# Jannertje/spacetime-fullgrid-parallel

Hardware: AMD Instinct MI355X
Metric: Kronecker-matvec GB/s (algorithmic bytes; share of 8 TB/s HBM peak in roofline.frac) + PCG iters/s, J_time=6 J_space=9 square (higher is better)
Workload: dtype f64; 1 GPU; y = (A_t kron M_x + M_t kron A_x) x, P1 on the uniform interval x P1 on the red-refined square, x ~ U[0,1) seed 128; J_space=9, N=65, M=1046529, nnz_M_x=7317521, nnz_A_x=5228553, parallelism=time-slab x1

## Files before the change

include/stk.h:

```cpp
#ifndef STK_H
#define STK_H

#include <stdint.h>

#ifdef __cplusplus
extern "C" {
#endif

const char *stk_last_error(void);
int stk_version(void);
int stk_device_info(int32_t *n_cu, int32_t *wave_size, int64_t *hbm_bytes);
int stk_set_tuning(const char *key, int32_t value);

int stk_slab_gather_columns(void *stream, int32_t M, int32_t n_cols,
                            const int32_t *cols, const double *x, int32_t ld_x,
                            double *y, int32_t ld_y);
int stk_slab_scatter_columns(void *stream, int32_t M, int32_t n_cols,
                             const int32_t *cols, const double *x, int32_t ld_x,
                             double *y, int32_t ld_y);

int stk_slab_ld(int32_t n_loc);
int stk_slab_alloc(int32_t M, int32_t n_loc, int32_t *ld, double **slab);
int stk_slab_free(double *slab);
int stk_slab_upload(void *stream, int32_t M, int32_t n_loc, int32_t ld,
// ... 298 lines not shown
    const int32_t *fwd_rows;
    int32_t n_bwd;
    const int32_t *bwd_ptr_host;
    const int32_t *bwd_rows;
    const int32_t *p_indptr, *p_indices;
    const double *p_vals;
    const int32_t *r_indptr, *r_indices;
    const double *r_vals;
    const stk_ell_rows *ell_a, *ell_fwd, *ell_bwd, *ell_p, *ell_r;
    const int32_t *fwd_pos_host, *bwd_pos_host;
    const stk_ell_rows *ell_ra;
    const stk_ell_rows *ell_fwd0;
    int32_t n_tile_rows;
    const int32_t *fwd_tile_row_host, *bwd_tile_row_host;
    const stk_ell_rows *ell_fwd_alt, *ell_bwd_alt;
} stk_mg_level;

typedef struct stk_mg stk_mg;

int stk_mg_create(int32_t n_levels, const stk_mg_level *levels_host,
                  int32_t smoothsteps, int32_t vcycles, int32_t n_kinds,
                  const double *coarse_inv, int32_t max_ld, stk_mg **out);
int stk_mg_destroy(stk_mg *mg);
int stk_mg_set_option(stk_mg *plan, const char *key, int32_t value);
int stk_mg_apply(stk_mg *mg, void *stream, int32_t n_loc, int32_t ld,
                 double ca, const double *cm, const int32_t *kind,
                 const double *f, double *u);
int stk_mg_coarse_levels(const stk_mg *plan);
int stk_mg_set_member_matrices(stk_mg *plan, int32_t level, int32_t n_kinds,
                               const int32_t *const *indptr_host,
// ... 119 lines not shown
```

spacetime-fullgrid-parallel_amd/csrc/mg.hip:

```cpp
#include <algorithm>
#include <cstdio>
#include <cstdlib>
#include <cstring>
#include <map>
#include <vector>

#include "stk_common.h"

namespace {

constexpr int GBS = 256;

__global__ __launch_bounds__(GBS) void gs_group_kernel(int64_t total, const int32_t *__restrict__ rows,
                                                       int32_t n_loc, int32_t ld,
                                                       const int32_t *__restrict__ indptr,
                                                       const int32_t *__restrict__ indices,
                                                       const double *__restrict__ va, double ca,
                                                       const double *__restrict__ vm,
                                                       const double *__restrict__ cm,
                                                       const int32_t *__restrict__ diag,
                                                       const double *__restrict__ f, double *u, int diag_free)
{
    const int64_t stride = (int64_t)gridDim.x * GBS;
    for (int64_t idx = (int64_t)blockIdx.x * GBS + threadIdx.x; idx < total; idx += stride) {
// ... 39 lines not shown

}

constexpr int64_t COARSE_MAX_ROWS = 4096;

struct EllLevel {
    bool has_a = false, has_gs = false, has_p = false, has_r = false, has_ra = false, has_alt = false;
    bool ra_rows_as_r = false;
    stk_ell_rows a, fwd, bwd, p, r, ra;
    stk_ell_rows fwd_alt, bwd_alt;
    std::vector<stk_ell_rows> fwd0;
    std::vector<int32_t> fwd_pos, bwd_pos;
    std::vector<int32_t> fwd_trow, bwd_trow;
    int n_tile_rows = 0;
    mutable std::map<int, std::vector<int32_t>> fwd_strips, bwd_strips;
};

struct stk_mg {
    std::vector<stk_mg_level> lv;
    std::vector<EllLevel> ell;
    std::vector<std::vector<int32_t>> fwd_ptr, bwd_ptr;
    int smoothsteps, vcycles, n_kinds, max_ld;
    const double *coarse_inv;
    std::vector<double *> u, f, r;
    stk_coarse_plan *coarse = nullptr;
    int Lc = -1;
    std::vector<void *> adopted;
    int fuse_restrict = -1;
    int fuse_min_level = 0, fuse_max_level = 1 << 30;
    int fast_until_cycle = 0;
    int fast_parts = 0;
    int strip_pct = 100;
};

static inline bool ell_slab_ok(int64_t rows, int ld)
{
    return (ld & 1) == 0 && rows * ld * 8 < ((int64_t)1 << 36);
}

static bool can_zero_start(const stk_mg *mg, int level, int ld)
{
    const EllLevel &E = mg->ell[level];
    return stk_tune(g_tuning.mg_zero_start) && level >= 1 && mg->smoothsteps >= 1 && E.has_gs && !E.fwd0.empty() &&
           E.fwd0.size() + 1 == E.fwd_pos.size() && ell_slab_ok(mg->lv[level].n, ld);
}

static const std::vector<int32_t> *strip_table(const EllLevel &E, bool backward, int64_t rows, int ld, int its,
// ... 8 lines not shown
    const int T = E.n_tile_rows, span = T + Q - 1;
    const int strip_width = stk_tune(g_tuning.mg_strip_width);
    const int min_width = strip_width > 0 ? strip_width * Q : 2;
    if (S > span / min_width) S = span / min_width;
    if (S < 2) return nullptr;
    auto &cache = backward ? E.bwd_strips : E.fwd_strips;
    const int key = S * 1024 + its;
    auto it = cache.find(key);
    if (it != cache.end()) return &it->second;
    const std::vector<int32_t> &tr = backward ? E.bwd_trow : E.fwd_trow;
    std::vector<int32_t> tab((size_t)S * Q * 2);
    for (int s = 0; s < S; ++s)
        for (int q = 0; q < Q; ++q) {
            const int g = q % ng;
            const int32_t *b = tr.data() + pos[g], *e = tr.data() + pos[g + 1];
            const int lo_row = (int)((int64_t)s * span / S) - q, hi_row = (int)((int64_t)(s + 1) * span / S) - q;
            const int32_t *lo = (s == 0) ? b : std::lower_bound(b, e, lo_row);
            const int32_t *hi = (s == S - 1) ? e : std::lower_bound(b, e, hi_row);
            tab[((size_t)s * Q + q) * 2] = (int32_t)(lo - tr.data());
            tab[((size_t)s * Q + q) * 2 + 1] = (int32_t)(hi - tr.data());
        }
    return &cache.emplace(key, std::move(tab)).first->second;
}

static int smooth_level(stk_mg *mg, hipStream_t st, int level, int n_loc, int ld, double ca, const double *cm,
                        int its, bool backward, const double *f, double *u, bool zero_start = false, int cycle = 1 << 30)
{
    const stk_mg_level &L = mg->lv[level];
    const EllLevel &E = mg->ell[level];
    if (E.has_gs && ell_slab_ok(L.n, ld)) {
        const bool alt = E.has_alt && cycle < mg->fast_until_cycle;
        const stk_ell_rows &e = alt ? (backward ? E.bwd_alt : E.fwd_alt) : (backward ? E.bwd : E.fwd);
        const std::vector<int32_t> &pos = backward ? E.bwd_pos : E.fwd_pos;
        const int ng = (int)pos.size() - 1;
        const bool zs = zero_start && !backward && its >= 1;
        const std::vector<int32_t> *strips =
            strip_table(E, backward, L.n, ld, its, stk_tune(g_tuning.mg_strip_mb) * (mg->strip_pct / 100.0));
        const int S = strips ? (int)(strips->size() / (2 * (size_t)ng * its)) : 1;
        const int Q = its * ng;
        for (int s = 0; s < S; ++s)
            for (int q = 0; q < Q; ++q) {
                const int g = q % ng;
                const int p0 = strips ? (*strips)[((size_t)s * Q + q) * 2] : pos[g];
                const int p1 = strips ? (*strips)[((size_t)s * Q + q) * 2 + 1] : pos[g + 1];
                if (strips) g_tuning.mg_strips_used.fetch_add(1, std::memory_order_relaxed);
                int rc;
                if (zs && q < ng) {
                    rc = stk_rows_ell_launch(st, 1, &E.fwd0[g], p0 - pos[g], p1 - pos[g], n_loc, ld, L.n, L.n, ca, cm,
                                             g == 0 ? f : u, 0.0, 0.0, f, u, 1);
                } else {
                    rc = stk_rows_ell_launch(st, 1, &e, p0, p1, n_loc, ld, L.n, L.n, ca, cm, u, 0.0, 0.0, f, u);
                }
                if (rc) return rc;
            }
        return 0;
    }
    const std::vector<int32_t> &ptr = backward ? mg->bwd_ptr[level] : mg->fwd_ptr[level];
    const int32_t *rows = backward ? L.bwd_rows : L.fwd_rows;
    const int ngroups = (int)ptr.size() - 1;
    for (int it = 0; it < its; ++it) {
        for (int g = 0; g < ngroups; ++g) {
            const int nr = ptr[g + 1] - ptr[g];
            if (nr == 0) continue;
            const int64_t total = (int64_t)nr * n_loc;
            hipLaunchKernelGGL(gs_group_kernel, dim3(stk_flat_grid(total, GBS)), dim3(GBS), 0, st, total,
                               rows + ptr[g], n_loc, ld, L.indptr, L.indices, L.vals_a, ca,
                               cm ? L.vals_m : nullptr, cm, L.diag, f, u, E.has_gs ? E.fwd.diag_free : 1);
            STK_LAUNCH_CHECK();
        }
    }
    return 0;
// ... 12 lines not shown
    if (u_zero && j >= 1 && !zero_start) {
        const int cols = std::min(ld, (n_loc + 1) & ~1);
        if (cols == ld)
            STK_HIP(hipMemsetAsync(u_j, 0, sizeof(double) * (size_t)L.n * ld, st));
        else
            STK_HIP(hipMemset2DAsync(u_j, sizeof(double) * (size_t)ld, 0, sizeof(double) * (size_t)cols, (size_t)L.n,
                                     st));
    }
    if (j == 0) {
        const int total = L.n * n_loc;
        hipLaunchKernelGGL(coarse_kernel, dim3((total + GBS - 1) / GBS), dim3(GBS), 0, st, L.n, n_loc, ld,
                           mg->coarse_inv, cm ? 1.0 : 1.0 / ca, cm ? kind : nullptr, f_j, u_j);
        STK_LAUNCH_CHECK();
        return 0;
    }
    int rc = smooth_level(mg, st, j, n_loc, ld, ca, cm, mg->smoothsteps, false, f_j, u_j, zero_start,
                          (mg->fast_parts & 1) ? -1 : cycle);
    if (rc) return rc;
    const stk_mg_level &C = mg->lv[j - 1];
    double *r_j = mg->r[j], *d_c = mg->f[j - 1], *u_c = mg->u[j - 1];
    const EllLevel &E = mg->ell[j];
    const bool even = ell_slab_ok(L.n, ld);
    const bool fuse_restrict = (mg->fuse_restrict >= 0 ? mg->fuse_restrict != 0 : stk_tune(g_tuning.mg_fuse_restrict) != 0) &&
                               ((j >= mg->fuse_min_level && j <= mg->fuse_max_level) || cycle < mg->fast_until_cycle ||
                                (mg->fast_parts & 2));
    if (fuse_restrict && E.has_ra && E.has_r && even) {
        const int one_pass = stk_tune(g_tuning.mg_restrict_one_pass);
        rc = (one_pass && E.ra_rows_as_r && (cm != nullptr || one_pass >= 2))
                 ? stk_rows_ell2_launch(st, &E.ra, &E.r, n_loc, ld, L.n, C.n, ca, cm, u_j, f_j, d_c)
                 : -1;
        if (rc == -1) {
            rc = stk_rows_ell_launch(st, 0, &E.r, 0, E.r.n_pos, n_loc, ld, L.n, C.n, 1.0, nullptr, f_j, 1.0, 0.0,
                                     nullptr, d_c);
            if (rc) return rc;
            rc = stk_rows_ell_launch(st, 0, &E.ra, 0, E.ra.n_pos, n_loc, ld, L.n, C.n, ca, cm, u_j, 1.0, -1.0, d_c,
                                     d_c);
        }
        if (rc) return rc;
    } else {
        if (E.has_a && even)
            rc = stk_rows_ell_launch(st, 0, &E.a, 0, E.a.n_pos, n_loc, ld, L.n, L.n, ca, cm, u_j, 1.0, -1.0, f_j,
                                     r_j);
        else
            rc = stk_csr_spmm(st, L.n, n_loc, ld, L.indptr, L.indices, L.vals_a, ca, cm ? L.vals_m : nullptr, cm,
                              u_j, 1.0, -1.0, f_j, r_j);
        if (rc) return rc;
        if (E.has_r && even)
            rc = stk_rows_ell_launch(st, 0, &E.r, 0, E.r.n_pos, n_loc, ld, L.n, C.n, 1.0, nullptr, r_j, 1.0, 0.0,
                                     nullptr, d_c);
        else
            rc = stk_csr_spmm(st, C.n, n_loc, ld, L.r_indptr, L.r_indices, L.r_vals, 1.0, nullptr, nullptr, r_j,
                              1.0, 0.0, nullptr, d_c);
        if (rc) return rc;
    }
    rc = mgm(mg, st, j - 1, n_loc, ld, ca, cm, kind, d_c, u_c, true, cycle);
    if (rc) return rc;
    if (E.has_p && even)
        rc = stk_rows_ell_launch(st, 0, &E.p, 0, E.p.n_pos, n_loc, ld, C.n, L.n, 1.0, nullptr, u_c, -1.0, 1.0, u_j,
                                 u_j);
    else
        rc = stk_csr_spmm(st, L.n, n_loc, ld, L.p_indptr, L.p_indices, L.p_vals, 1.0, nullptr, nullptr, u_c, -1.0,
                          1.0, u_j, u_j);
    if (rc) return rc;
    return smooth_level(mg, st, j, n_loc, ld, ca, cm, mg->smoothsteps, true, f_j, u_j, false, cycle);
}

extern "C" int stk_mg_create(int32_t n_levels, const stk_mg_level *levels, int32_t smoothsteps, int32_t vcycles,
                             int32_t n_kinds, const double *coarse_inv, int32_t max_ld, stk_mg **out)
{
    STK_REQUIRE(n_levels >= 1 && levels && out, "stk_mg_create: bad arguments");
    STK_REQUIRE(smoothsteps >= 0 && vcycles >= 1 && max_ld >= 1, "stk_mg_create: bad parameters");
    STK_REQUIRE(coarse_inv && n_kinds >= 1, "stk_mg_create: coarse inverse missing");
    stk_mg *mg = new stk_mg();
    mg->smoothsteps = smoothsteps;
    mg->vcycles = vcycles;
    mg->n_kinds = n_kinds;
    mg->max_ld = max_ld;
    mg->coarse_inv = coarse_inv;
    mg->lv.assign(levels, levels + n_levels);
// ... 26 lines not shown
            E.fwd_pos.assign(L.fwd_pos_host, L.fwd_pos_host + L.n_fwd + 1);
            E.bwd_pos.assign(L.bwd_pos_host, L.bwd_pos_host + L.n_bwd + 1);
            E.has_gs = true;
        }
        if (E.has_gs && L.ell_fwd_alt && L.ell_bwd_alt && L.ell_fwd_alt->n_pos == E.fwd.n_pos &&
            L.ell_bwd_alt->n_pos == E.bwd.n_pos) {
            E.fwd_alt = *L.ell_fwd_alt;
            E.bwd_alt = *L.ell_bwd_alt;
            E.has_alt = true;
        }
        if (E.has_gs && L.n_tile_rows > 1 && L.fwd_tile_row_host && L.bwd_tile_row_host) {
            E.fwd_trow.assign(L.fwd_tile_row_host, L.fwd_tile_row_host + E.fwd.n_pos);
            E.bwd_trow.assign(L.bwd_tile_row_host, L.bwd_tile_row_host + E.bwd.n_pos);
            E.n_tile_rows = L.n_tile_rows;
        }
        mg->lv[j].ell_a = mg->lv[j].ell_fwd = mg->lv[j].ell_bwd = mg->lv[j].ell_p = mg->lv[j].ell_r = nullptr;
        mg->lv[j].ell_ra = mg->lv[j].ell_fwd0 = nullptr;
        mg->lv[j].ell_fwd_alt = mg->lv[j].ell_bwd_alt = nullptr;
    }
    mg->u.assign(n_levels, nullptr);
    mg->f.assign(n_levels, nullptr);
    mg->r.assign(n_levels, nullptr);
    for (int j = 0; j < n_levels; ++j) {
        const stk_mg_level &L = mg->lv[j];
        if (L.n <= 0 || !L.indptr || !L.indices || !L.vals_a || !L.diag) {
            stk_set_error("stk_mg_create: level %d incomplete", j);
            stk_mg_destroy(mg);
            return 2;
        }
        if (j > 0) {
// ... 105 lines not shown
        mg->fuse_min_level = value;
        return 0;
    }
    if (std::strcmp(key, "fuse_restrict_max_level") == 0) {
        mg->fuse_max_level = value;
        return 0;
    }
    if (std::strcmp(key, "fast_until_cycle") == 0) {
        mg->fast_until_cycle = value;
        return 0;
    }
    if (std::strcmp(key, "fast_parts") == 0) {
        mg->fast_parts = value;
        return 0;
    }
    if (std::strcmp(key, "strip_pct") == 0) {
        STK_REQUIRE(value >= 1 && value <= 10000, "stk_mg_set_option: strip_pct=%d not in 1..10000", value);
        mg->strip_pct = value;
        return 0;
    }
    stk_set_error("stk_mg_set_option: unknown key '%s' (fuse_restrict, fuse_restrict_min_level, fuse_restrict_max_level, fast_until_cycle, fast_parts, strip_pct)", key);
    return 2;
}

extern "C" int stk_mg_apply(stk_mg *mg, void *stream, int32_t n_loc, int32_t ld, double ca, const double *cm,
                            const int32_t *kind, const double *f, double *u)
{
    const stk_timed timed_(STK_OP_MULTIGRID, stream);
    STK_REQUIRE(mg && f && u && f != u, "stk_mg_apply: bad pointers");
    STK_REQUIRE(n_loc > 0 && ld >= n_loc && ld <= mg->max_ld, "stk_mg_apply: ld=%d exceeds plan max_ld=%d", ld,
                mg->max_ld);
    STK_REQUIRE(cm == nullptr || mg->lv[0].vals_m != nullptr, "stk_mg_apply: cm given but plan has no vals_m");
    STK_REQUIRE(ca != 0.0 || cm, "stk_mg_apply: zero matrix");
    hipStream_t st = stk_stream(stream);
    const int J = (int)mg->lv.size() - 1;
    for (int v = 0; v < mg->vcycles; ++v) {
// ... 16 lines not shown
```

spacetime-fullgrid-parallel_amd/csrc/rows_ell.hip:

```cpp
#include <cstring>

#include "stk_common.h"

namespace {

constexpr int BS = 512;
enum { MODE_SPMM = 0, MODE_GS = 1 };

struct RowsArgs {
    const int32_t *idx;
    const double *va, *vm;
    const int32_t *row_ids;
    const double *dia_a, *dia_m;
    const double *cm;
    const double *x;
    const double *z;
    double *y;
    double ca, alpha, beta;
    int32_t pos_begin, pos_end;
    int32_t n_loc, ld, P, R;
    int32_t ngroups, chunk;
    int32_t reverse;
    int32_t zero_own;
    uint32_t x_bytes, y_bytes;
// ... 369 lines not shown
        case 9: return launch_npf<MODE, 9, HAS_M>(st, a, grid, lds);
        case 12: return launch_npf<MODE, 12, HAS_M>(st, a, grid, lds);
        case 16: return launch_npf<MODE, 16, HAS_M>(st, a, grid, lds);
        case 20: return launch_npf<MODE, 20, HAS_M>(st, a, grid, lds);
    }
    stk_set_error("rows_ell: K=%d is not one of 2, 4, 5, 6, 7, 9, 12, 16, 20", K);
    return 2;
}

}

int stk_rows_ell_launch(hipStream_t st, int mode, const stk_ell_rows *e, int32_t pos_begin, int32_t pos_end,
                        int32_t n_loc, int32_t ld, int64_t x_rows, int64_t y_rows, double ca, const double *cm,
                        const double *x, double alpha, double beta, const double *z, double *y, int zero_own)
{
    if (pos_end <= pos_begin) return 0;
    STK_REQUIRE(e && e->idx && e->va, "rows_ell: incomplete matrix");
    STK_REQUIRE((cm == nullptr) || e->vm, "rows_ell: cm given but the matrix has no vm");
    STK_REQUIRE(n_loc > 0 && ld >= n_loc && (ld & 1) == 0, "rows_ell: bad n_loc=%d ld=%d (ld must be even)", n_loc,
                ld);
    STK_REQUIRE(x_rows * ld * 8 < ((int64_t)1 << 36) && y_rows * ld * 8 < ((int64_t)1 << 36),
                "rows_ell: slab exceeds 64 GiB");
    STK_REQUIRE((((uintptr_t)x | (uintptr_t)y | (uintptr_t)z) & 15) == 0, "rows_ell: slabs must be 16-byte aligned");
    STK_REQUIRE((n_loc + 1) / 2 <= BS, "rows_ell: n_loc too large");
    RowsArgs a;
    a.idx = e->idx;
    a.va = e->va;
    a.vm = cm ? e->vm : nullptr;
    a.row_ids = e->row_ids;
    a.dia_a = e->dia_a;
    a.dia_m = e->dia_m;
    a.cm = cm;
// ... 5 lines not shown
    a.beta = z ? beta : 0.0;
    a.pos_begin = pos_begin;
    a.pos_end = pos_end;
    a.n_loc = n_loc;
    a.ld = ld;
    a.P = (n_loc + 1) / 2;
    a.R = BS / a.P;
    if (a.R * e->K > 4 * BS) a.R = 4 * BS / e->K;
    a.ngroups = (pos_end - pos_begin + a.R - 1) / a.R;
    a.chunk = (a.ngroups + 7) / 8;
    a.reverse = (int)(g_rows_launch_count++ & 1u);
    a.zero_own = (zero_own || e->diag_free) ? 1 : 0;
    a.wide = stk_tune(g_tuning.rows_force_wide) || x_rows * ld * 8 >= ((int64_t)1 << 32) || y_rows * ld * 8 >= ((int64_t)1 << 32);
    a.x_bytes = a.wide ? 0u : (uint32_t)(x_rows * ld * 8);
    a.y_bytes = a.wide ? 0u : (uint32_t)(y_rows * ld * 8);
    a.nt_store = mode == MODE_GS ? 0 : 1;
    if (mode == MODE_GS) STK_REQUIRE(e->dia_a && (!cm || e->dia_m), "rows_ell: GS needs the diagonal arrays");
    const int K = e->K;
    const int KS = (K + 3) & ~3;
    const bool has_m = cm != nullptr;
    const size_t buf_doubles =
        ((size_t)(has_m ? 2 : 1) * a.R * KS + 2 * a.R + ((size_t)a.R * KS + a.R + 1) / 2 + 2) & ~(size_t)1;
    const size_t lds = 2 * buf_doubles * sizeof(double) + 16;
    const int n_cu = stk_cu_count();
    int per_cu = K >= 12 ? 2 : 3;
    int per_xcd = (n_cu / 8) * per_cu;
    if (per_xcd > a.chunk) per_xcd = a.chunk;
    if (per_xcd < 1) per_xcd = 1;
    const unsigned grid = (unsigned)per_xcd * 8;
    if (mode == MODE_GS)
        return has_m ? launch_k<MODE_GS, true>(st, a, K, grid, lds) : launch_k<MODE_GS, false>(st, a, K, grid, lds);
    return has_m ? launch_k<MODE_SPMM, true>(st, a, K, grid, lds) : launch_k<MODE_SPMM, false>(st, a, K, grid, lds);
}

int stk_rows_ell2_launch(hipStream_t st, const stk_ell_rows *e, const stk_ell_rows *e2, int32_t n_loc, int32_t ld,
                         int64_t x_rows, int64_t y_rows, double ca, const double *cm, const double *x,
                         const double *x2, double *y)
{
    if (e->K != 20 || e2->K != 7 || e->n_pos != e2->n_pos || e->n_pos <= 0) return -1;
    STK_REQUIRE(e->idx && e->va && e2->idx && e2->va, "rows_ell2: incomplete matrix");
    STK_REQUIRE((cm == nullptr) || e->vm, "rows_ell2: cm given but the matrix has no vm");
    STK_REQUIRE(n_loc > 0 && ld >= n_loc && (ld & 1) == 0, "rows_ell2: bad n_loc=%d ld=%d", n_loc, ld);
    STK_REQUIRE(x_rows * ld * 8 < ((int64_t)1 << 36) && y_rows * ld * 8 < ((int64_t)1 << 36), "rows_ell2: slab exceeds 64 GiB");
    STK_REQUIRE((((uintptr_t)x | (uintptr_t)x2 | (uintptr_t)y) & 15) == 0, "rows_ell2: slabs must be 16-byte aligned");
    STK_REQUIRE((n_loc + 1) / 2 <= BS, "rows_ell2: n_loc too large");
    constexpr int K = 20, K2 = 7, KS = 20, KS2 = 8;
    Rows2Args b;
    RowsArgs &a = b.a;
    a.idx = e->idx;
    a.va = e->va;
    a.vm = cm ? e->vm : nullptr;
    a.row_ids = e->row_ids;
    a.dia_a = a.dia_m = nullptr;
    a.cm = cm;
    a.x = x;
    a.z = y;
    a.y = y;
    a.ca = ca;
    a.alpha = 1.0;
    a.beta = 0.0;
    a.pos_begin = 0;
    a.pos_end = e->n_pos;
    a.n_loc = n_loc;
    a.ld = ld;
    a.P = (n_loc + 1) / 2;
    a.R = BS / a.P;
    if (a.R * K > 4 * BS) a.R = 4 * BS / K;
    a.ngroups = (e->n_pos + a.R - 1) / a.R;
    a.chunk = (a.ngroups + 7) / 8;
    a.reverse = (int)(g_rows_launch_count++ & 1u);
    a.zero_own = 0;
    a.wide = stk_tune(g_tuning.rows_force_wide) || x_rows * ld * 8 >= ((int64_t)1 << 32) || y_rows * ld * 8 >= ((int64_t)1 << 32);
    a.x_bytes = a.wide ? 0u : (uint32_t)(x_rows * ld * 8);
    a.y_bytes = a.wide ? 0u : (uint32_t)(y_rows * ld * 8);
    a.nt_store = 0;
    b.idx2 = e2->idx;
    b.va2 = e2->va;
    b.x2 = x2;
    b.x2_bytes = a.x_bytes;
    const bool has_m = cm != nullptr;
    auto lds_of = [&](int R) {
        const size_t val_doubles = (size_t)(has_m ? 2 : 1) * R * KS + (size_t)R * KS2;
        const size_t buf_doubles = (val_doubles + ((size_t)R * KS + (size_t)R * KS2 + R + 1) / 2 + 2) & ~(size_t)1;
        return 2 * buf_doubles * sizeof(double) + 16;
    };
    while (a.R > 1 && lds_of(a.R) > 60 * 1024) --a.R;
    a.ngroups = (e->n_pos + a.R - 1) / a.R;
    a.chunk = (a.ngroups + 7) / 8;
    const size_t lds = lds_of(a.R);
    const int n_cu = stk_cu_count();
    int per_xcd = (n_cu / 8) * 2;
    if (per_xcd > a.chunk) per_xcd = a.chunk;
    if (per_xcd < 1) per_xcd = 1;
    const unsigned grid = (unsigned)per_xcd * 8;
    if (has_m)
        return a.wide ? launch2_npf<K, K2, true, true>(st, b, grid, lds) : launch2_npf<K, K2, true, false>(st, b, grid, lds);
    return a.wide ? launch2_npf<K, K2, false, true>(st, b, grid, lds) : launch2_npf<K, K2, false, false>(st, b, grid, lds);
}

extern "C" int stk_ell_spmm(void *stream, const stk_ell_rows *ell, int32_t n_loc, int32_t ld, int32_t x_rows,
                            double ca, const double *cm, const double *x, double alpha, double beta,
                            const double *z, double *y)
// ... 8 lines not shown
```

spacetime-fullgrid-parallel_amd/source/_lib.py:

```python
import ctypes
import os

import numpy as np
import torch

_HERE = os.path.dirname(os.path.abspath(__file__))
LIB_PATH = os.path.join(os.path.dirname(_HERE), 'libstk.so')

c_i32, c_i64, c_f64, c_p = (ctypes.c_int32, ctypes.c_int64, ctypes.c_double,
                            ctypes.c_void_p)


OPERATOR_FN = ctypes.CFUNCTYPE(ctypes.c_int, ctypes.c_void_p, ctypes.c_void_p,
                               ctypes.c_void_p, ctypes.c_void_p)
ALLREDUCE_FN = ctypes.CFUNCTYPE(ctypes.c_int, ctypes.c_void_p,
                                ctypes.POINTER(ctypes.c_double), ctypes.c_int32)


class EllPattern(ctypes.Structure):
    _fields_ = [('M', c_i32), ('K', c_i32), ('ell_idx', c_p),
                ('row_ids', c_p), ('ovf_indptr', c_p), ('ovf_indices', c_p)]


class KronEllTerm(ctypes.Structure):
# ... 33 lines not shown
                ('n_fwd', c_i32), ('fwd_ptr_host', c_p), ('fwd_rows', c_p),
                ('n_bwd', c_i32), ('bwd_ptr_host', c_p), ('bwd_rows', c_p),
                ('p_indptr', c_p), ('p_indices', c_p), ('p_vals', c_p),
                ('r_indptr', c_p), ('r_indices', c_p), ('r_vals', c_p),
                ('ell_a', ctypes.POINTER(EllRows)),
                ('ell_fwd', ctypes.POINTER(EllRows)),
                ('ell_bwd', ctypes.POINTER(EllRows)),
                ('ell_p', ctypes.POINTER(EllRows)),
                ('ell_r', ctypes.POINTER(EllRows)),
                ('fwd_pos_host', c_p), ('bwd_pos_host', c_p),
                ('ell_ra', ctypes.POINTER(EllRows)),
                ('ell_fwd0', ctypes.POINTER(EllRows)),
                ('n_tile_rows', c_i32), ('fwd_tile_row_host', c_p),
                ('bwd_tile_row_host', c_p),
                ('ell_fwd_alt', ctypes.POINTER(EllRows)),
                ('ell_bwd_alt', ctypes.POINTER(EllRows))]


_PROTOTYPES = {
    'stk_last_error': (ctypes.c_char_p, []),
    'stk_version': (ctypes.c_int, []),
    'stk_device_info': (ctypes.c_int, [c_p, c_p, c_p]),
    'stk_axpby': (ctypes.c_int, [c_p, c_i64, c_f64, c_p, c_f64, c_p]),
    'stk_axpbyz': (ctypes.c_int, [c_p, c_i64, c_f64, c_p, c_f64, c_p, c_p]),
    'stk_dot_work_size': (c_i64, []),
    'stk_dot': (ctypes.c_int, [c_p, c_i64, c_p, c_p, c_p, c_p]),
    'stk_set_tuning': (ctypes.c_int, [ctypes.c_char_p, c_i32]),
    'stk_partition': (ctypes.c_int, [c_i32, c_i32, c_i32, c_p, c_p, c_p, c_p]),
    'stk_pcg_work_size': (c_i64, [c_i64]),
    'stk_pcg_solve': (ctypes.c_int, [
        c_p, c_i64, OPERATOR_FN, c_p, OPERATOR_FN, c_p, ALLREDUCE_FN, c_p, c_p,
# ... 303 lines not shown
```

spacetime-fullgrid-parallel_amd/source/multigrid.py:

```python
import ctypes
import threading

import numpy as np
import scipy.sparse as sp
import torch

from . import _lib
from .assembly import prolongation_matrices
from .linop import (EllRowsMatrix, SpaceOp, tile_order_from_coords,
                    tile_rows_from_coords,
                    union_pattern)


class MeshHierarchy:
    def __init__(self, fes=None, shared_comm=None, P_mats=None):
        self.coords = None
        if P_mats is None:
            mesh = getattr(fes, 'mesh', fes)
            P_mats = prolongation_matrices(mesh)
            self.coords = mesh.points[~mesh.boundary]
        self.shared_comm = shared_comm
        self.P_mats = [sp.csr_matrix(P) for P in P_mats]
        self.R_mats = [P.T.tocsr() for P in self.P_mats]
        self.J = len(self.P_mats)
# ... 17 lines not shown
    def tile_order(self, n):
        if self.coords is None:
            return np.arange(n, dtype=np.int32)
        return self.shared(('tile', n), lambda: tile_order_from_coords(self.coords[:n]))

    def coord_band(self, n):
        if self.coords is None:
            return None

        def make():
            _, band = np.unique(np.round(np.asarray(self.coords)[:n, -1], 12), return_inverse=True)
            return band.astype(np.int64)

        return self.shared(('band', n), make)

    def transfer_copies(self, j):
        def make():
            P = sp.csr_matrix(self.P_mats[j - 1])
            R = sp.csr_matrix(self.R_mats[j - 1])
            dev, ells = {}, {}
            for name, m, order in (('p', P, self.tile_order(P.shape[0])),
                                   ('r', R, self.tile_order(P.shape[1]))):
                m.sort_indices()
                dev[name + '_indptr'] = _lib.to_dev(np.asarray(m.indptr, dtype=np.int32))
                dev[name + '_indices'] = _lib.to_dev(np.asarray(m.indices, dtype=np.int32))
                dev[name + '_vals'] = _lib.to_dev(np.asarray(m.data, dtype=np.float64))
                ells[name] = EllRowsMatrix(m.indptr, m.indices, m.data, None, order)
            return dev, ells

        return self.shared(('transfer', j), make)

    def prepare(self):
        sizes = [P.shape[1] for P in self.P_mats] + ([self.P_mats[-1].shape[0]] if self.P_mats else [])
        for n in reversed(sizes):
            self.tile_order(n)
            self.coord_band(n)
        if _lib.compute_device().type == 'cuda':
            for j in reversed(range(1, self.J + 1)):
                self.transfer_copies(j)
        return self


def _tile_order(hierarchy, n):
    if hasattr(hierarchy, 'tile_order'):
        return hierarchy.tile_order(n)
    coords = getattr(hierarchy, 'coords', None)
    return np.arange(n, dtype=np.int32) if coords is None else tile_order_from_coords(coords[:n])


def _shared(hierarchy, key, make):
    return hierarchy.shared(key, make) if hasattr(hierarchy, 'shared') else make()


def _mat_key(mat):
    return (mat.indptr.ctypes.data, mat.indices.ctypes.data, mat.data.ctypes.data, mat.nnz)


def _drop_roundoff(mat, rel=1e-14):
    if mat.nnz:
        mat.data[np.abs(mat.data) < rel * np.abs(mat.data).max()] = 0.0
        mat.eliminate_zeros()
    return mat
# ... 296 lines not shown
        if self.has_m:
            dev['vals_m'] = _lib.to_dev(vals[1])
        L.n = n
        host = {}
        if j > 0:
            tile = _tile_order(hierarchy, n)
            rank = np.empty(n, dtype=np.int64)
            rank[tile] = np.arange(n)
            band = coupling_bands(hierarchy.coords, indptr, indices, rows_of,
                                  hierarchy.coord_band(n) if hasattr(hierarchy, 'coord_band') else None)
            if band is not None and self.band_merge > 1 and hierarchy.coords is not None:
                band = band // self.band_merge
            key = rank if band is None else band * np.int64(n) + rank
            vm = vals[1] if self.has_m else None
            moved = {}
            transfers = threading.Thread(
                target=_lib.in_device_context(self._transfer_ells),
                args=(j, hierarchy, mats, tile, moved))
            transfers.start()
            ells = {'a': EllRowsMatrix(indptr, indices, vals[0], vm, tile)}
            for name, bw in (('fwd', False), ('bwd', True)):
                ptr, rows = gauss_seidel_schedule(indptr, indices, bw,
                                                  on_device=(dev['indptr'], dev['indices']))
                host[name + '_ptr'] = ptr
                dev[name + '_rows'] = _lib.to_dev(rows)
                setattr(L, 'n_' + name, len(ptr) - 1)
                setattr(L, name + '_ptr_host',
                        ptr.ctypes.data_as(ctypes.c_void_p))
                groups = [rows[ptr[g]:ptr[g + 1]] for g in range(len(ptr) - 1)]
                groups = [r_[np.argsort(key[r_], kind='stable')] for r_ in groups]
                listed = (np.concatenate(groups) if n else
                          np.zeros(0, dtype=np.int64))
                full_rows, alt_copies = self._row_form(j)
                if not full_rows:
                    ells[name] = EllRowsMatrix(indptr, indices, vals[0], vm,
# ... 13 lines not shown
                host[name + '_pos'] = ptr
                setattr(L, name + '_pos_host',
                        ptr.ctypes.data_as(ctypes.c_void_p))
                if not bw:
                    fwd_groups = groups
            transfers.join()
            if 'error' in moved:
                raise moved['error']
            dev.update(moved['dev'])
            ells.update(moved['ells'])
            if all(e.ok for e in ells.values()):
                if moved['ra'].ok:
                    ells['ra'] = moved['ra']
                for name, e in ells.items():
                    setattr(L, 'ell_' + name, ctypes.pointer(e.struct))
                host['ells'] = ells
                self._zero_start_ells(L, host, indptr, indices, vals[0], vm,
                                      diag, fwd_groups)
                EllRowsMatrix.check_all(list(ells.values()) + list(host.get('fwd0', ([],))[0]))
        for name, t in dev.items():
            setattr(L, name, _lib.ptr(t))
        self._keep.append((dev, host))
        if j == self.J:
            self.groups_fwd = len(host['fwd_ptr']) - 1 if j > 0 else 0

    def _transfer_ells(self, j, hierarchy, mats, tile, out):
        try:
            P = sp.csr_matrix(hierarchy.P_mats[j - 1])
            R = sp.csr_matrix(hierarchy.R_mats[j - 1])
            nc = P.shape[1]
            tile_c = _tile_order(hierarchy, nc)

            def transfer_copies():
                dev_, ells_ = {}, {}
                for name, m, order in (('p', P, tile), ('r', R, tile_c)):
                    m.sort_indices()
                    dev_[name + '_indptr'] = _lib.to_dev(np.asarray(m.indptr, dtype=np.int32))
                    dev_[name + '_indices'] = _lib.to_dev(np.asarray(m.indices, dtype=np.int32))
                    dev_[name + '_vals'] = _lib.to_dev(np.asarray(m.data, dtype=np.float64))
                    ells_[name] = EllRowsMatrix(m.indptr, m.indices, m.data, None, order)
                return dev_, ells_

            if hasattr(hierarchy, 'transfer_copies'):
                shared_dev, shared_ells = hierarchy.transfer_copies(j)
            else:
                shared_dev, shared_ells = transfer_copies()
            dev, ells = dict(shared_dev), dict(shared_ells)
            prods = [_shared(hierarchy, ('ra', j, _mat_key(m)),
                             lambda m=m: _drop_roundoff(galerkin_product(R, m, None))) for m in mats]
            ra_ptr, ra_idx, ra_vals = union_pattern(prods)
            out['ra'] = EllRowsMatrix(ra_ptr, ra_idx, ra_vals[0],
                                      ra_vals[1] if self.has_m else None, tile_c)
            out['dev'], out['ells'] = dev, ells
        except Exception as exc:
            out['error'] = exc

    def _zero_start_ells(self, L, host, indptr, indices, va, vm, diag,
                         groups):
        n = len(indptr) - 1
        if not groups or any(len(g) == 0 for g in groups):
            return
        grp = np.empty(n, dtype=np.int64)
        for g, rows in enumerate(groups):
            grp[rows] = g
        rows_of = np.repeat(np.arange(n), np.diff(indptr))
        kept = np.bincount(rows_of[grp[indices] < grp[rows_of]], minlength=n)
        ells = [EllRowsMatrix(indptr, indices, va, vm, rows, pad_col=-1,
# ... 268 lines not shown
```

Baseline: 4264 GB/s.

## Interleave restriction and prolongation with Gauss-Seidel strips for cache reuse

```diff
diff --git a/include/stk.h b/include/stk.h
--- a/include/stk.h
+++ b/include/stk.h
@@ -336,6 +336,7 @@
     int32_t n_tile_rows;
     const int32_t *fwd_tile_row_host, *bwd_tile_row_host;
     const stk_ell_rows *ell_fwd_alt, *ell_bwd_alt;
+    const int32_t *a_ready_host, *r_ready_host, *ra_ready_host, *p_band_host;
 } stk_mg_level;
 
 typedef struct stk_mg stk_mg;
diff --git a/spacetime-fullgrid-parallel_amd/csrc/mg.hip b/spacetime-fullgrid-parallel_amd/csrc/mg.hip
--- a/spacetime-fullgrid-parallel_amd/csrc/mg.hip
+++ b/spacetime-fullgrid-parallel_amd/csrc/mg.hip
@@ -2,10 +2,12 @@
 #include <cstdio>
 #include <cstdlib>
 #include <cstring>
+#include <functional>
 #include <map>
 #include <vector>
 
-#include "stk_common.h"
+#include "mg_strips.h"
+#include "rows_ell.h"
 
 namespace {
 
@@ -77,6 +79,7 @@
     std::vector<int32_t> fwd_trow, bwd_trow;
     int n_tile_rows = 0;
     mutable std::map<int, std::vector<int32_t>> fwd_strips, bwd_strips;
+    std::vector<int32_t> a_ready, r_ready, ra_ready, p_band;
 };
 
 struct stk_mg {
@@ -94,6 +97,7 @@
     int fast_until_cycle = 0;
     int fast_parts = 0;
     int strip_pct = 100;
+    int strip_transfers = 1;
 };
 
 static inline bool ell_slab_ok(int64_t rows, int ld)
@@ -132,7 +136,7 @@
         for (int q = 0; q < Q; ++q) {
             const int g = q % ng;
             const int32_t *b = tr.data() + pos[g], *e = tr.data() + pos[g + 1];
-            const int lo_row = (int)((int64_t)s * span / S) - q, hi_row = (int)((int64_t)(s + 1) * span / S) - q;
+            const int lo_row = stk_strip_edge(s, T, Q, S) - q, hi_row = stk_strip_edge(s + 1, T, Q, S) - q;
             const int32_t *lo = (s == 0) ? b : std::lower_bound(b, e, lo_row);
             const int32_t *hi = (s == S - 1) ? e : std::lower_bound(b, e, hi_row);
             tab[((size_t)s * Q + q) * 2] = (int32_t)(lo - tr.data());
@@ -141,8 +145,22 @@
     return &cache.emplace(key, std::move(tab)).first->second;
 }
 
+static const std::vector<int32_t> *level_strips(const stk_mg *mg, int level, int ld, int its, bool backward)
+{
+    const EllLevel &E = mg->ell[level];
+    if (!E.has_gs || !ell_slab_ok(mg->lv[level].n, ld)) return nullptr;
+    return strip_table(E, backward, mg->lv[level].n, ld, its,
+                       stk_tune(g_tuning.mg_strip_mb) * (mg->strip_pct / 100.0));
+}
+
+struct StripHooks {
+    const std::vector<int32_t> *strips;
+    std::function<int(int, int)> before, after;
+};
+
 static int smooth_level(stk_mg *mg, hipStream_t st, int level, int n_loc, int ld, double ca, const double *cm,
-                        int its, bool backward, const double *f, double *u, bool zero_start = false, int cycle = 1 << 30)
+                        int its, bool backward, const double *f, double *u, bool zero_start = false, int cycle = 1 << 30,
+                        const StripHooks *hooks = nullptr)
 {
     const stk_mg_level &L = mg->lv[level];
     const EllLevel &E = mg->ell[level];
@@ -152,11 +170,14 @@
         const std::vector<int32_t> &pos = backward ? E.bwd_pos : E.fwd_pos;
         const int ng = (int)pos.size() - 1;
         const bool zs = zero_start && !backward && its >= 1;
-        const std::vector<int32_t> *strips =
-            strip_table(E, backward, L.n, ld, its, stk_tune(g_tuning.mg_strip_mb) * (mg->strip_pct / 100.0));
+        const std::vector<int32_t> *strips = hooks ? hooks->strips : level_strips(mg, level, ld, its, backward);
         const int S = strips ? (int)(strips->size() / (2 * (size_t)ng * its)) : 1;
         const int Q = its * ng;
-        for (int s = 0; s < S; ++s)
+        for (int s = 0; s < S; ++s) {
+            if (hooks && hooks->before) {
+                const int rc = hooks->before(s, S);
+                if (rc) return rc;
+            }
             for (int q = 0; q < Q; ++q) {
                 const int g = q % ng;
                 const int p0 = strips ? (*strips)[((size_t)s * Q + q) * 2] : pos[g];
@@ -171,8 +192,14 @@
                 }
                 if (rc) return rc;
             }
-        return 0;
-    }
+            if (hooks && hooks->after) {
+                const int rc = hooks->after(s, S);
+                if (rc) return rc;
+            }
+        }
+        return 0;
+    }
+    STK_REQUIRE(!hooks, "smooth_level: strip hooks on a level without ELL sweeps");
     const std::vector<int32_t> &ptr = backward ? mg->bwd_ptr[level] : mg->fwd_ptr[level];
     const int32_t *rows = backward ? L.bwd_rows : L.fwd_rows;
     const int ngroups = (int)ptr.size() - 1;
@@ -215,47 +242,99 @@
         STK_LAUNCH_CHECK();
         return 0;
     }
-    int rc = smooth_level(mg, st, j, n_loc, ld, ca, cm, mg->smoothsteps, false, f_j, u_j, zero_start,
-                          (mg->fast_parts & 1) ? -1 : cycle);
-    if (rc) return rc;
     const stk_mg_level &C = mg->lv[j - 1];
     double *r_j = mg->r[j], *d_c = mg->f[j - 1], *u_c = mg->u[j - 1];
     const EllLevel &E = mg->ell[j];
     const bool even = ell_slab_ok(L.n, ld);
+    const int its = mg->smoothsteps, T = E.n_tile_rows;
     const bool fuse_restrict = (mg->fuse_restrict >= 0 ? mg->fuse_restrict != 0 : stk_tune(g_tuning.mg_fuse_restrict) != 0) &&
                                ((j >= mg->fuse_min_level && j <= mg->fuse_max_level) || cycle < mg->fast_until_cycle ||
                                 (mg->fast_parts & 2));
-    if (fuse_restrict && E.has_ra && E.has_r && even) {
-        const int one_pass = stk_tune(g_tuning.mg_restrict_one_pass);
-        rc = (one_pass && E.ra_rows_as_r && (cm != nullptr || one_pass >= 2))
-                 ? stk_rows_ell2_launch(st, &E.ra, &E.r, n_loc, ld, L.n, C.n, ca, cm, u_j, f_j, d_c)
-                 : -1;
-        if (rc == -1) {
-            rc = stk_rows_ell_launch(st, 0, &E.r, 0, E.r.n_pos, n_loc, ld, L.n, C.n, 1.0, nullptr, f_j, 1.0, 0.0,
-                                     nullptr, d_c);
+    const bool fused = fuse_restrict && E.has_ra && E.has_r && even;
+    const int one_pass_key = stk_tune(g_tuning.mg_restrict_one_pass);
+    const bool one_pass = fused && one_pass_key && E.ra_rows_as_r && (cm != nullptr || one_pass_key >= 2) &&
+                          stk_rows_ell2_has(&E.ra, &E.r);
+    const bool two_step_ell = !fused && E.has_a && E.has_r && even;
+    auto restricted_residual = [&](int a0, int a1, int p0, int p1, int store) -> int {
+        if (one_pass)
+            return stk_rows_ell2_run(st, &E.ra, &E.r, p0, p1, n_loc, ld, L.n, C.n, ca, cm, u_j, f_j, d_c);
+        int rc;
+        if (fused) {
+            rc = stk_rows_ell_run(st, 0, &E.r, p0, p1, n_loc, ld, L.n, C.n, 1.0, nullptr, f_j, 1.0, 0.0, nullptr, d_c,
+                                  0, store);
             if (rc) return rc;
-            rc = stk_rows_ell_launch(st, 0, &E.ra, 0, E.ra.n_pos, n_loc, ld, L.n, C.n, ca, cm, u_j, 1.0, -1.0, d_c,
-                                     d_c);
-        }
+            return stk_rows_ell_run(st, 0, &E.ra, p0, p1, n_loc, ld, L.n, C.n, ca, cm, u_j, 1.0, -1.0, d_c, d_c, 0,
+                                    STK_STORE_STREAM);
+        }
+        rc = stk_rows_ell_run(st, 0, &E.a, a0, a1, n_loc, ld, L.n, L.n, ca, cm, u_j, 1.0, -1.0, f_j, r_j, 0, store);
+        if (rc) return rc;
+        return stk_rows_ell_run(st, 0, &E.r, p0, p1, n_loc, ld, L.n, C.n, 1.0, nullptr, r_j, 1.0, 0.0, nullptr, d_c, 0,
+                                STK_STORE_STREAM);
+    };
+
+    const std::vector<int32_t> *pre = nullptr;
+    if (mg->strip_transfers && its >= 1 && T > 1 &&
+        (fused ? !E.ra_ready.empty() && (one_pass || E.ra_rows_as_r) : two_step_ell && !E.a_ready.empty() && !E.r_ready.empty()))
+        pre = level_strips(mg, j, ld, its, false);
+    const int pre_cycle = (mg->fast_parts & 1) ? -1 : cycle;
+    int rc;
+    if (pre) {
+        const int Q = its * ((int)E.fwd_pos.size() - 1), S = (int)(pre->size() / (2 * (size_t)Q));
+        std::vector<int32_t> cut, cut_a;
+        if (fused) {
+            stk_strip_cuts_descending(E.ra_ready.data(), E.ra.n_pos, T, Q, S, cut);
+        } else {
+            stk_strip_cuts_descending(E.a_ready.data(), E.a.n_pos, T, Q, S, cut_a);
+            stk_strip_cuts_descending(E.r_ready.data(), E.r.n_pos, T, Q, S, cut);
+        }
+        StripHooks hooks;
+        hooks.strips = pre;
+        hooks.after = [&](int s, int) -> int {
+            g_tuning.mg_strips_used.fetch_add(one_pass ? 1 : 2, std::memory_order_relaxed);
+            return restricted_residual(fused ? 0 : cut_a[s], fused ? 0 : cut_a[s + 1], cut[s], cut[s + 1], STK_STORE_KEEP);
+        };
+        rc = smooth_level(mg, st, j, n_loc, ld, ca, cm, its, false, f_j, u_j, zero_start, pre_cycle, &hooks);
         if (rc) return rc;
     } else {
-        if (E.has_a && even)
-            rc = stk_rows_ell_launch(st, 0, &E.a, 0, E.a.n_pos, n_loc, ld, L.n, L.n, ca, cm, u_j, 1.0, -1.0, f_j,
-                                     r_j);
-        else
-            rc = stk_csr_spmm(st, L.n, n_loc, ld, L.indptr, L.indices, L.vals_a, ca, cm ? L.vals_m : nullptr, cm,
-                              u_j, 1.0, -1.0, f_j, r_j);
+        rc = smooth_level(mg, st, j, n_loc, ld, ca, cm, its, false, f_j, u_j, zero_start, pre_cycle);
         if (rc) return rc;
-        if (E.has_r && even)
-            rc = stk_rows_ell_launch(st, 0, &E.r, 0, E.r.n_pos, n_loc, ld, L.n, C.n, 1.0, nullptr, r_j, 1.0, 0.0,
-                                     nullptr, d_c);
-        else
-            rc = stk_csr_spmm(st, C.n, n_loc, ld, L.r_indptr, L.r_indices, L.r_vals, 1.0, nullptr, nullptr, r_j,
-                              1.0, 0.0, nullptr, d_c);
+        if (fused || two_step_ell) {
+            rc = restricted_residual(0, E.a.n_pos, 0, E.r.n_pos, STK_STORE_STREAM);
+        } else {
+            if (E.has_a && even)
+                rc = stk_rows_ell_launch(st, 0, &E.a, 0, E.a.n_pos, n_loc, ld, L.n, L.n, ca, cm, u_j, 1.0, -1.0, f_j,
+                                         r_j);
+            else
+                rc = stk_csr_spmm(st, L.n, n_loc, ld, L.indptr, L.indices, L.vals_a, ca, cm ? L.vals_m : nullptr, cm,
+                                  u_j, 1.0, -1.0, f_j, r_j);
+            if (rc) return rc;
+            if (E.has_r && even)
+                rc = stk_rows_ell_launch(st, 0, &E.r, 0, E.r.n_pos, n_loc, ld, L.n, C.n, 1.0, nullptr, r_j, 1.0, 0.0,
+                                         nullptr, d_c);
+            else
+                rc = stk_csr_spmm(st, C.n, n_loc, ld, L.r_indptr, L.r_indices, L.r_vals, 1.0, nullptr, nullptr, r_j,
+                                  1.0, 0.0, nullptr, d_c);
+        }
         if (rc) return rc;
     }
     rc = mgm(mg, st, j - 1, n_loc, ld, ca, cm, kind, d_c, u_c, true, cycle);
     if (rc) return rc;
+    const std::vector<int32_t> *post = nullptr;
+    if (mg->strip_transfers && its >= 1 && T > 1 && E.has_p && even && !E.p_band.empty())
+        post = level_strips(mg, j, ld, its, true);
+    if (post) {
+        const int Q = its * ((int)E.bwd_pos.size() - 1), S = (int)(post->size() / (2 * (size_t)Q));
+        std::vector<int32_t> cut;
+        stk_strip_cuts_ascending(E.p_band.data(), E.p.n_pos, T, Q, S, cut);
+        StripHooks hooks;
+        hooks.strips = post;
+        hooks.before = [&](int s, int) -> int {
+            g_tuning.mg_strips_used.fetch_add(1, std::memory_order_relaxed);
+            return stk_rows_ell_run(st, 0, &E.p, cut[s], cut[s + 1], n_loc, ld, C.n, L.n, 1.0, nullptr, u_c, -1.0, 1.0,
+                                    u_j, u_j, 0, STK_STORE_KEEP);
+        };
+        return smooth_level(mg, st, j, n_loc, ld, ca, cm, its, true, f_j, u_j, false, cycle, &hooks);
+    }
     if (E.has_p && even)
         rc = stk_rows_ell_launch(st, 0, &E.p, 0, E.p.n_pos, n_loc, ld, C.n, L.n, 1.0, nullptr, u_c, -1.0, 1.0, u_j,
                                  u_j);
@@ -263,7 +342,7 @@
         rc = stk_csr_spmm(st, L.n, n_loc, ld, L.p_indptr, L.p_indices, L.p_vals, 1.0, nullptr, nullptr, u_c, -1.0,
                           1.0, u_j, u_j);
     if (rc) return rc;
-    return smooth_level(mg, st, j, n_loc, ld, ca, cm, mg->smoothsteps, true, f_j, u_j, false, cycle);
+    return smooth_level(mg, st, j, n_loc, ld, ca, cm, its, true, f_j, u_j, false, cycle);
 }
 
 extern "C" int stk_mg_create(int32_t n_levels, const stk_mg_level *levels, int32_t smoothsteps, int32_t vcycles,
@@ -320,6 +399,20 @@
             E.bwd_trow.assign(L.bwd_tile_row_host, L.bwd_tile_row_host + E.bwd.n_pos);
             E.n_tile_rows = L.n_tile_rows;
         }
+        if (E.n_tile_rows > 1) {
+            const int T = E.n_tile_rows;
+            auto take = [T](std::vector<int32_t> &dst, const int32_t *src, bool has, int32_t n_pos, bool up = true) {
+                if (!has || !src) return;
+                dst.assign(src, src + n_pos);
+                const int32_t lag = up ? stk_strip_envelope_up(dst) : stk_strip_envelope_down(dst);
+                if (4 * (int64_t)lag > T) dst.clear();
+            };
+            if (E.has_a && L.a_ready_host && std::is_sorted(L.a_ready_host, L.a_ready_host + E.a.n_pos))
+                E.a_ready.assign(L.a_ready_host, L.a_ready_host + E.a.n_pos);
+            take(E.r_ready, L.r_ready_host, E.has_r && !E.a_ready.empty(), E.r.n_pos);
+            take(E.ra_ready, L.ra_ready_host, E.has_ra, E.ra.n_pos);
+            take(E.p_band, L.p_band_host, E.has_p, E.p.n_pos, false);
+        }
         mg->lv[j].ell_a = mg->lv[j].ell_fwd = mg->lv[j].ell_bwd = mg->lv[j].ell_p = mg->lv[j].ell_r = nullptr;
         mg->lv[j].ell_ra = mg->lv[j].ell_fwd0 = nullptr;
         mg->lv[j].ell_fwd_alt = mg->lv[j].ell_bwd_alt = nullptr;
@@ -455,12 +548,16 @@
         mg->fast_parts = value;
         return 0;
     }
+    if (std::strcmp(key, "strip_transfers") == 0) {
+        mg->strip_transfers = value != 0;
+        return 0;
+    }
     if (std::strcmp(key, "strip_pct") == 0) {
         STK_REQUIRE(value >= 1 && value <= 10000, "stk_mg_set_option: strip_pct=%d not in 1..10000", value);
         mg->strip_pct = value;
         return 0;
     }
-    stk_set_error("stk_mg_set_option: unknown key '%s' (fuse_restrict, fuse_restrict_min_level, fuse_restrict_max_level, fast_until_cycle, fast_parts, strip_pct)", key);
+    stk_set_error("stk_mg_set_option: unknown key '%s' (fuse_restrict, fuse_restrict_min_level, fuse_restrict_max_level, fast_until_cycle, fast_parts, strip_pct, strip_transfers)", key);
     return 2;
 }
 
diff --git a/spacetime-fullgrid-parallel_amd/csrc/mg_strips.h b/spacetime-fullgrid-parallel_amd/csrc/mg_strips.h
--- /dev/null
+++ b/spacetime-fullgrid-parallel_amd/csrc/mg_strips.h
@@ -0,0 +1,61 @@
+#ifndef STK_MG_STRIPS_H
+#define STK_MG_STRIPS_H
+
+#include <algorithm>
+#include <cstdint>
+#include <vector>
+
+static inline int32_t stk_strip_edge(int s, int T, int Q, int S)
+{
+    return (int32_t)((int64_t)s * (T + Q - 1) / S);
+}
+
+static inline int32_t stk_strip_envelope_up(std::vector<int32_t> &v)
+{
+    int32_t lift = 0;
+    for (size_t p = 1; p < v.size(); ++p) {
+        if (v[p] < v[p - 1]) {
+            lift = std::max(lift, v[p - 1] - v[p]);
+            v[p] = v[p - 1];
+        }
+    }
+    return lift;
+}
+
+static inline int32_t stk_strip_envelope_down(std::vector<int32_t> &v)
+{
+    int32_t drop = 0;
+    for (size_t p = v.size(); p-- > 1;) {
+        if (v[p - 1] > v[p]) {
+            drop = std::max(drop, v[p - 1] - v[p]);
+            v[p - 1] = v[p];
+        }
+    }
+    return drop;
+}
+
+static inline void stk_strip_cuts_descending(const int32_t *ready, int32_t n_pos, int T, int Q, int S,
+                                             std::vector<int32_t> &cut)
+{
+    cut.assign((size_t)S + 1, 0);
+    for (int s = 0; s + 1 < S; ++s) {
+        const int32_t bound = stk_strip_edge(s + 1, T, Q, S) - (Q - 1);
+        const int32_t c = (int32_t)(std::lower_bound(ready, ready + n_pos, bound) - ready);
+        cut[(size_t)s + 1] = std::max(c, cut[(size_t)s]);
+    }
+    cut[(size_t)S] = n_pos;
+}
+
+static inline void stk_strip_cuts_ascending(const int32_t *band, int32_t n_pos, int T, int Q, int S,
+                                            std::vector<int32_t> &cut)
+{
+    cut.assign((size_t)S + 1, 0);
+    for (int s = 0; s + 1 < S; ++s) {
+        const int32_t bound = stk_strip_edge(s + 1, T, Q, S);
+        const int32_t c = (int32_t)(std::upper_bound(band, band + n_pos, bound) - band);
+        cut[(size_t)s + 1] = std::max(c, cut[(size_t)s]);
+    }
+    cut[(size_t)S] = n_pos;
+}
+
+#endif
diff --git a/spacetime-fullgrid-parallel_amd/csrc/rows_ell.h b/spacetime-fullgrid-parallel_amd/csrc/rows_ell.h
--- /dev/null
+++ b/spacetime-fullgrid-parallel_amd/csrc/rows_ell.h
@@ -0,0 +1,19 @@
+#ifndef STK_ROWS_ELL_H
+#define STK_ROWS_ELL_H
+
+#include "stk_common.h"
+
+enum { STK_STORE_STREAM = 0, STK_STORE_KEEP = 1 };
+
+int stk_rows_ell_run(hipStream_t st, int mode, const stk_ell_rows *e, int32_t pos_begin, int32_t pos_end,
+                     int32_t n_loc, int32_t ld, int64_t x_rows, int64_t y_rows, double ca, const double *cm,
+                     const double *x, double alpha, double beta, const double *z, double *y, int zero_own,
+                     int store);
+
+bool stk_rows_ell2_has(const stk_ell_rows *e, const stk_ell_rows *e2);
+
+int stk_rows_ell2_run(hipStream_t st, const stk_ell_rows *e, const stk_ell_rows *e2, int32_t pos_begin,
+                      int32_t pos_end, int32_t n_loc, int32_t ld, int64_t x_rows, int64_t y_rows, double ca,
+                      const double *cm, const double *x, const double *x2, double *y);
+
+#endif
diff --git a/spacetime-fullgrid-parallel_amd/csrc/rows_ell.hip b/spacetime-fullgrid-parallel_amd/csrc/rows_ell.hip
--- a/spacetime-fullgrid-parallel_amd/csrc/rows_ell.hip
+++ b/spacetime-fullgrid-parallel_amd/csrc/rows_ell.hip
@@ -1,6 +1,6 @@
 #include <cstring>
 
-#include "stk_common.h"
+#include "rows_ell.h"
 
 namespace {
 
@@ -407,8 +407,18 @@
                         int32_t n_loc, int32_t ld, int64_t x_rows, int64_t y_rows, double ca, const double *cm,
                         const double *x, double alpha, double beta, const double *z, double *y, int zero_own)
 {
+    return stk_rows_ell_run(st, mode, e, pos_begin, pos_end, n_loc, ld, x_rows, y_rows, ca, cm, x, alpha, beta, z, y,
+                            zero_own, STK_STORE_STREAM);
+}
+
+int stk_rows_ell_run(hipStream_t st, int mode, const stk_ell_rows *e, int32_t pos_begin, int32_t pos_end,
+                     int32_t n_loc, int32_t ld, int64_t x_rows, int64_t y_rows, double ca, const double *cm,
+                     const double *x, double alpha, double beta, const double *z, double *y, int zero_own, int store)
+{
     if (pos_end <= pos_begin) return 0;
     STK_REQUIRE(e && e->idx && e->va, "rows_ell: incomplete matrix");
+    STK_REQUIRE(pos_begin >= 0 && pos_end <= e->n_pos, "rows_ell: positions %d..%d of %d", pos_begin, pos_end,
+                e->n_pos);
     STK_REQUIRE((cm == nullptr) || e->vm, "rows_ell: cm given but the matrix has no vm");
     STK_REQUIRE(n_loc > 0 && ld >= n_loc && (ld & 1) == 0, "rows_ell: bad n_loc=%d ld=%d (ld must be even)", n_loc,
                 ld);
@@ -444,7 +454,7 @@
     a.wide = stk_tune(g_tuning.rows_force_wide) || x_rows * ld * 8 >= ((int64_t)1 << 32) || y_rows * ld * 8 >= ((int64_t)1 << 32);
     a.x_bytes = a.wide ? 0u : (uint32_t)(x_rows * ld * 8);
     a.y_bytes = a.wide ? 0u : (uint32_t)(y_rows * ld * 8);
-    a.nt_store = mode == MODE_GS ? 0 : 1;
+    a.nt_store = (mode == MODE_GS || store == STK_STORE_KEEP) ? 0 : 1;
     if (mode == MODE_GS) STK_REQUIRE(e->dia_a && (!cm || e->dia_m), "rows_ell: GS needs the diagonal arrays");
     const int K = e->K;
     const int KS = (K + 3) & ~3;
@@ -467,7 +477,22 @@
                          int64_t x_rows, int64_t y_rows, double ca, const double *cm, const double *x,
                          const double *x2, double *y)
 {
-    if (e->K != 20 || e2->K != 7 || e->n_pos != e2->n_pos || e->n_pos <= 0) return -1;
+    return stk_rows_ell2_run(st, e, e2, 0, e->n_pos, n_loc, ld, x_rows, y_rows, ca, cm, x, x2, y);
+}
+
+bool stk_rows_ell2_has(const stk_ell_rows *e, const stk_ell_rows *e2)
+{
+    return e->K == 20 && e2->K == 7 && e->n_pos == e2->n_pos && e->n_pos > 0;
+}
+
+int stk_rows_ell2_run(hipStream_t st, const stk_ell_rows *e, const stk_ell_rows *e2, int32_t pos_begin,
+                      int32_t pos_end, int32_t n_loc, int32_t ld, int64_t x_rows, int64_t y_rows, double ca,
+                      const double *cm, const double *x, const double *x2, double *y)
+{
+    if (!stk_rows_ell2_has(e, e2)) return -1;
+    STK_REQUIRE(pos_begin >= 0 && pos_end <= e->n_pos, "rows_ell2: positions %d..%d of %d", pos_begin, pos_end,
+                e->n_pos);
+    if (pos_end <= pos_begin) return 0;
     STK_REQUIRE(e->idx && e->va && e2->idx && e2->va, "rows_ell2: incomplete matrix");
     STK_REQUIRE((cm == nullptr) || e->vm, "rows_ell2: cm given but the matrix has no vm");
     STK_REQUIRE(n_loc > 0 && ld >= n_loc && (ld & 1) == 0, "rows_ell2: bad n_loc=%d ld=%d", n_loc, ld);
@@ -489,14 +514,14 @@
     a.ca = ca;
     a.alpha = 1.0;
     a.beta = 0.0;
-    a.pos_begin = 0;
-    a.pos_end = e->n_pos;
+    a.pos_begin = pos_begin;
+    a.pos_end = pos_end;
     a.n_loc = n_loc;
     a.ld = ld;
     a.P = (n_loc + 1) / 2;
     a.R = BS / a.P;
     if (a.R * K > 4 * BS) a.R = 4 * BS / K;
-    a.ngroups = (e->n_pos + a.R - 1) / a.R;
+    a.ngroups = (pos_end - pos_begin + a.R - 1) / a.R;
     a.chunk = (a.ngroups + 7) / 8;
     a.reverse = (int)(g_rows_launch_count++ & 1u);
     a.zero_own = 0;
@@ -515,7 +540,7 @@
         return 2 * buf_doubles * sizeof(double) + 16;
     };
     while (a.R > 1 && lds_of(a.R) > 60 * 1024) --a.R;
-    a.ngroups = (e->n_pos + a.R - 1) / a.R;
+    a.ngroups = (pos_end - pos_begin + a.R - 1) / a.R;
     a.chunk = (a.ngroups + 7) / 8;
     const size_t lds = lds_of(a.R);
     const int n_cu = stk_cu_count();
diff --git a/spacetime-fullgrid-parallel_amd/source/_lib.py b/spacetime-fullgrid-parallel_amd/source/_lib.py
--- a/spacetime-fullgrid-parallel_amd/source/_lib.py
+++ b/spacetime-fullgrid-parallel_amd/source/_lib.py
@@ -71,7 +71,9 @@
                 ('n_tile_rows', c_i32), ('fwd_tile_row_host', c_p),
                 ('bwd_tile_row_host', c_p),
                 ('ell_fwd_alt', ctypes.POINTER(EllRows)),
-                ('ell_bwd_alt', ctypes.POINTER(EllRows))]
+                ('ell_bwd_alt', ctypes.POINTER(EllRows)),
+                ('a_ready_host', c_p), ('r_ready_host', c_p),
+                ('ra_ready_host', c_p), ('p_band_host', c_p)]
 
 
 _PROTOTYPES = {
diff --git a/spacetime-fullgrid-parallel_amd/source/multigrid.py b/spacetime-fullgrid-parallel_amd/source/multigrid.py
--- a/spacetime-fullgrid-parallel_amd/source/multigrid.py
+++ b/spacetime-fullgrid-parallel_amd/source/multigrid.py
@@ -55,13 +55,32 @@
 
         return self.shared(('band', n), make)
 
+    def band_order(self, n):
+        if self.coords is None:
+            return self.tile_order(n)
+
+        def make():
+            tile = self.tile_order(n)
+            rank = np.empty(n, dtype=np.int64)
+            rank[tile] = np.arange(n)
+            band = self.coord_band(n)
+            group = max(1, min(TRANSFER_BAND_ROWS, (int(band.max()) + 1) // 64))
+            return np.argsort((band // group) * np.int64(n) + rank, kind='stable').astype(np.int32)
+
+        return self.shared(('band_order', n), make)
+
+    def transfer_order(self, j):
+        P = self.P_mats[j - 1]
+        order = self.band_order if P.shape[0] > STRIP_LEVEL_ROWS else self.tile_order
+        return order(P.shape[0]), order(P.shape[1])
+
     def transfer_copies(self, j):
         def make():
             P = sp.csr_matrix(self.P_mats[j - 1])
             R = sp.csr_matrix(self.R_mats[j - 1])
             dev, ells = {}, {}
-            for name, m, order in (('p', P, self.tile_order(P.shape[0])),
-                                   ('r', R, self.tile_order(P.shape[1]))):
+            order_p, order_r = self.transfer_order(j)
+            for name, m, order in (('p', P, order_p), ('r', R, order_r)):
                 m.sort_indices()
                 dev[name + '_indptr'] = _lib.to_dev(np.asarray(m.indptr, dtype=np.int32))
                 dev[name + '_indices'] = _lib.to_dev(np.asarray(m.indices, dtype=np.int32))
@@ -76,6 +95,8 @@
         for n in reversed(sizes):
             self.tile_order(n)
             self.coord_band(n)
+            if n > STRIP_LEVEL_ROWS:
+                self.band_order(n)
         if _lib.compute_device().type == 'cuda':
             for j in reversed(range(1, self.J + 1)):
                 self.transfer_copies(j)
@@ -87,6 +108,22 @@
         return hierarchy.tile_order(n)
     coords = getattr(hierarchy, 'coords', None)
     return np.arange(n, dtype=np.int32) if coords is None else tile_order_from_coords(coords[:n])
+
+
+STRIP_LEVEL_ROWS = 4096
+TRANSFER_BAND_ROWS = 4
+
+
+def _transfer_order(hierarchy, j, tile, tile_c):
+    if hasattr(hierarchy, 'transfer_order'):
+        return hierarchy.transfer_order(j)
+    return tile, tile_c
+
+
+def _row_max(indptr, values, n):
+    if n == 0 or (np.diff(indptr) == 0).any():
+        return None
+    return np.maximum.reduceat(values, indptr[:-1])
 
 
 def _shared(hierarchy, key, make):
@@ -413,11 +450,16 @@
             key = rank if band is None else band * np.int64(n) + rank
             vm = vals[1] if self.has_m else None
             moved = {}
+            order_a = tile
+            if band is not None and n > STRIP_LEVEL_ROWS and hasattr(hierarchy, 'band_order'):
+                order_a = hierarchy.band_order(n)
+            moved['order_a'], moved['band'] = order_a, band
+            moved['row_ready'] = _row_max(indptr, band[indices], n) if order_a is not tile else None
             transfers = threading.Thread(
                 target=_lib.in_device_context(self._transfer_ells),
                 args=(j, hierarchy, mats, tile, moved))
             transfers.start()
-            ells = {'a': EllRowsMatrix(indptr, indices, vals[0], vm, tile)}
+            ells = {'a': EllRowsMatrix(indptr, indices, vals[0], vm, order_a)}
             for name, bw in (('fwd', False), ('bwd', True)):
                 ptr, rows = gauss_seidel_schedule(indptr, indices, bw,
                                                   on_device=(dev['indptr'], dev['indices']))
@@ -461,6 +503,9 @@
                     ells['ra'] = moved['ra']
                 for name, e in ells.items():
                     setattr(L, 'ell_' + name, ctypes.pointer(e.struct))
+                for name, arr in moved.get('ready', {}).items():
+                    host[name] = np.ascontiguousarray(arr, dtype=np.int32)
+                    setattr(L, name + '_host', host[name].ctypes.data_as(ctypes.c_void_p))
                 host['ells'] = ells
                 self._zero_start_ells(L, host, indptr, indices, vals[0], vm,
                                       diag, fwd_groups)
@@ -476,11 +521,11 @@
             P = sp.csr_matrix(hierarchy.P_mats[j - 1])
             R = sp.csr_matrix(hierarchy.R_mats[j - 1])
             nc = P.shape[1]
-            tile_c = _tile_order(hierarchy, nc)
+            order_p, order_c = _transfer_order(hierarchy, j, tile, _tile_order(hierarchy, nc))
 
             def transfer_copies():
                 dev_, ells_ = {}, {}
-                for name, m, order in (('p', P, tile), ('r', R, tile_c)):
+                for name, m, order in (('p', P, order_p), ('r', R, order_c)):
                     m.sort_indices()
                     dev_[name + '_indptr'] = _lib.to_dev(np.asarray(m.indptr, dtype=np.int32))
                     dev_[name + '_indices'] = _lib.to_dev(np.asarray(m.indices, dtype=np.int32))
@@ -497,7 +542,21 @@
                              lambda m=m: _drop_roundoff(galerkin_product(R, m, None))) for m in mats]
             ra_ptr, ra_idx, ra_vals = union_pattern(prods)
             out['ra'] = EllRowsMatrix(ra_ptr, ra_idx, ra_vals[0],
-                                      ra_vals[1] if self.has_m else None, tile_c)
+                                      ra_vals[1] if self.has_m else None, order_c)
+            band, row_ready = out['band'], out['row_ready']
+            if band is not None and row_ready is not None:
+                R.sort_indices()
+                a_ready = np.maximum.accumulate(row_ready[out['order_a']])
+                ran_with = np.empty_like(a_ready)
+                ran_with[out['order_a']] = a_ready
+                ready = {'a_ready': a_ready, 'p_band': band[order_p]}
+                ra_ready = _row_max(ra_ptr, band[ra_idx], nc)
+                r_ready = _row_max(R.indptr, ran_with[R.indices], nc)
+                if ra_ready is not None:
+                    ready['ra_ready'] = ra_ready[order_c]
+                if r_ready is not None:
+                    ready['r_ready'] = r_ready[order_c]
+                out['ready'] = ready
             out['dev'], out['ells'] = dev, ells
         except Exception as exc:
             out['error'] = exc
```

Result: no change. 4264 GB/s (-0.0%).
